# InSilicoModellingGroup/rdcFEs

Measured on AMD Instinct MI355X. Metric: elements_assembled_per_sec, higher is better.
Workload: dtype f64; 1 GPU; PIHNA TET4 K(119): 10110954 tets, 1728000 nodes, 5 unknowns, params run/PIHNA/input.dat (shipped), order=lex, state of SURVEY App. C (background (0,0,0,7170,0) of the shipped field file, tumour values inside a sphere r = 0.25; see state_sensitivity); scatter=rowgather, kernel_variant=auto, parallelism=single GPU, rank0_local_elements=10110954, rank0_nnz=639395950

## Files before the change

rdcfes_amd/csrc/rdc_capi.hip:

```cpp
#include <algorithm>
#include <cmath>
#include <cstdarg>
#include <cstdio>
#include <cstring>
#include <new>
#include <type_traits>

#include "rdc_internal.h"
#include "rdc_tet4_pihna_moments.h"
#include "rdc_tet4_ev.h"
#include "rdc_solid.h"

using namespace rdc;

namespace {

struct DevBuf {
  void* p = nullptr;
  size_t bytes = 0;
  bool owned = true;
};

thread_local char g_create_error[512] = "";

// ... 386 lines not shown
    a.rg2.sdesc = (const HostPrep::StoreDesc*)c->rg2_sdesc.p;
    a.rg2.contrib = (const uint16_t*)c->rg2_contrib.p;
    a.rg2.pair_aux = (const uint16_t*)c->rg2_aux.p;
    a.rg2.node_tab = (const uint16_t*)c->rg2_ntab.p;
    if (c->prep.rg4_nl_stride > 0) {
      a.rg2.nlist = (const uint32_t*)c->rg4_nlist.p;
      a.rg2.pair_loc = (const uint32_t*)c->rg4_ploc.p;
      a.rg2.nl_stride = c->prep.rg4_nl_stride;
      if ((M::NELEM > 0 || M::AUX_LOCAL_NODE >= 0) && !c->prep.pair_eid.empty()) {
        if (!c->rg5_eid_ready) {
          if ((rc = dev_upload(c, c->rg5_eid, c->prep.pair_eid))) return rc;
          c->rg5_eid_ready = true;
        }
        a.rg2.pair_eid = (const uint32_t*)c->rg5_eid.p;
      }
    }
    a.rg2.lds_bytes = c->prep.rg2_lds_bytes;
    a.rg2.block = c->prep.rg2_block;
  }
  const bool evc_model = EvcEligible<M>::value && evc_wanted(p, c->opt_special != 0);
  if (evc_model && a.nen == 4 && !c->ev_tried && c->prep.rg2_ok && c->opt_kernel == 0 && a.strategy == RDC_SCATTER_ROWGATHER && a.variant != RDC_VARIANT_GENERIC) {
    std::vector<uint32_t> conn_h((size_t)c->prep.n_elem * 4);
    RDC_HIP(c, hipMemcpyAsync(conn_h.data(), c->conn.p, conn_h.size() * sizeof(uint32_t), hipMemcpyDeviceToHost, c->stream));
    RDC_HIP(c, hipStreamSynchronize(c->stream));
    if ((rc = build_ev_lists(c, conn_h.data()))) return rc;
  }
  a.use_ev = c->prep_ev.ok && (c->opt_kernel == 0 || c->opt_kernel == 7) && c->opt_moments && (!c->opt_ablate || c->opt_kernel == 7) &&
             (!c->stamps.p || (c->opt_kernel == 7 && c->opt_ablate == 4)) && c->opt_occ != 1 && c->opt_ldspad == 0;
  a.opt_ev_occ = c->opt_ev_occ;
  a.opt_evc_occ = c->opt_evc_occ;
  a.opt_ev_resident = c->opt_ev_resident;
  a.opt_ev_bg = c->opt_ev_bg;
  if (c->opt_ev_resident) {
    if ((rc = dev_alloc(c, c->ev_ticket, 256))) return rc;
    a.ev_ticket = (int*)c->ev_ticket.p;
  }
  a.ev_grid = c->opt_grid > 0 ? c->opt_grid : 2 * c->n_cu;
  if (c->opt_kernel == 5 || c->opt_kernel == 7) a.opt_kernel = 0;
  if (a.use_ev) {
    a.ev.n_wg = (int)c->prep_ev.desc.size();
    a.ev.desc = (const HostPrepEv::Desc*)c->ev_desc.p;
    a.ev.nlist = (const uint32_t*)c->ev_nlist.p;
    a.ev.vloc = (const uint32_t*)c->ev_vloc.p;
    a.ev.vslot = (const uint32_t*)c->ev_vslot.p;
    a.ev.ntab = (const HostPrepEv::Node*)c->ev_ntab.p;
    a.ev.bpart = (const uint8_t*)c->ev_bpart.p;
    a.ev.nls = c->prep_ev.nls;
    a.ev.max_out_doubles = c->prep_ev.max_out_doubles;
  }
  bool hex_cl = false;
  if (a.nen == 8 && (M::NV == 3 || M::NV == 5) && c->opt_hex_kernel != 1 && (c->opt_part == 0 || c->opt_hex_kernel == 0) &&
      a.strategy == RDC_SCATTER_ROWGATHER && c->opt_solid_cl_waves == 31) {
    if ((rc = ensure_cluster_lists(c, 0))) return rc;
    hex_cl = c->solid_cl_state == 1;
  }
  bool pattern_ok = evc_model;
  if constexpr (std::is_same<M, Pihna>::value) pattern_ok = pihna_pattern_applies(p) || c->opt_ev_general;
  const bool ev_path = a.use_ev && (std::is_same<M, Pihna>::value || evc_model) && a.nen == 4 && a.variant != RDC_VARIANT_GENERIC &&
                       (c->opt_special || c->opt_ev_general || !std::is_same<M, Pihna>::value) && a.strategy == RDC_SCATTER_ROWGATHER && pattern_ok;
  if constexpr (std::is_same<M, Pihna>::value) a.ev_general = ev_path && c->opt_ev_general && !(c->opt_special && pihna_pattern_applies(p));
  if (!std::is_same<M, Pihna>::value) a.use_ev = ev_path && c->opt_kernel == 0;
  if (c->opt_part != 0 && ev_path) {
    if (c->opt_interior < 0) return fail(c, RDC_ERR_STATE, "\"part\" needs \"interior_nodes\"");
    if ((rc = ev_order_for_interior(c))) return rc;
    a.ev.wg_perm = (const uint32_t*)c->ev_perm.p;
    if (c->opt_part == 1) {
      c->part1_packed = false;
      c->part1_nodes = 0;
      if (c->ev_part1_wg == 0) return RDC_OK;
      c->part1_nodes = ev_part1_node_bound(c);
      a.ev.wg_begin = 0; a.ev.wg_count = c->ev_part1_wg;
      if (!c->pack_event) RDC_HIP(c, hipEventCreateWithFlags(&c->pack_event, hipEventDisableTiming));
      a.pack_part = 1; a.pack_event = c->pack_event;
      c->part1_packed = true;
    } else {
      a.ev.wg_begin = c->ev_part1_wg; a.ev.wg_count = -1;
      if (c->part1_packed) { a.pack_part = 2; a.pack_event = c->pack_event; }
      c->part1_packed = false;
    }
  } else
  if (c->opt_part != 0 && hex_cl) {
    c->part1_packed = false;
    if (c->opt_part == 1) {
      c->part1_nodes = c->scl_interior >= 0 ? c->scl_part1_nodes : 0;
      if (c->scl_interior < 0 || c->scl_n_wg_interior == 0) { c->part1_nodes = 0; return RDC_OK; }
    }
    a.cl = cluster_view(c, c->scl_interior >= 0 ? c->opt_part : (c->opt_part == 2 ? 0 : 1));
    if (a.cl.n_wg == 0) return RDC_OK;
  } else
  if (c->opt_part != 0) {
    const bool sub = a.nen == 4 && a.strategy == RDC_SCATTER_ROWGATHER && a.variant != RDC_VARIANT_GENERIC && a.rg2.n_wg > 0 &&
                     a.rg2.pair_aux && a.rg2.nlist && a.rg2.block == 256 && a.opt_kernel == 0 && c->opt_interior >= 0 &&
                     ((M::NELEM == 0 && M::AUX_LOCAL_NODE < 0) || a.rg2.pair_eid);
    const int split = sub ? part1_workgroups(c) : 0;
    if (c->opt_part == 1) {
      c->part1_packed = false;
      c->part1_nodes = 0;
      if (!sub || split == 0) return RDC_OK;
      c->part1_nodes = (int64_t)c->prep.wg2[(size_t)split - 1].n0 + c->prep.wg2[(size_t)split - 1].nnodes;
      a.rg2.wg_begin = 0; a.rg2.wg_count = split;
      if (!c->pack_event) RDC_HIP(c, hipEventCreateWithFlags(&c->pack_event, hipEventDisableTiming));
      a.pack_part = 1; a.pack_event = c->pack_event;
      c->part1_packed = true;
    } else {
      a.rg2.wg_begin = split; a.rg2.wg_count = -1;
      if (sub && c->part1_packed) { a.pack_part = 2; a.pack_event = c->pack_event; }
      c->part1_packed = false;
    }
  } else {
    c->part1_packed = false;
  }
  if (hex_cl && c->opt_part == 0) {
    a.cl = cluster_view(c);
    a.cl.grid = c->opt_hex_kernel == 2 ? 2 * c->n_cu : 0;
  }
  a.val = (double*)c->val.p;
  a.rhs = (double*)c->rhs.p;
  a.stream = c->stream;
  a.colour_ptr = c->prep.colour_ptr.data();
  a.n_colours = c->prep.n_colours;
  a.n_wg = c->prep.rowgather_ok ? (int)c->prep.wg_node_ptr.size() - 1 : 0;
  a.lds_bytes = c->prep.rg_lds_bytes;
  a.ev_start = nullptr;
  hipEvent_t ev_stop = nullptr;
  if (c->timing) {
    if ((rc = next_event_pair(c, &a.ev_start, &ev_stop))) return rc;
  }
  hipError_t e = launch_specialised<M>(a, k, *p);
  if (e != hipSuccess) return fail(c, RDC_ERR_HIP, "kernel launch failed: %s", hipGetErrorString(e));
  if (c->timing) RDC_HIP(c, hipEventRecord(ev_stop, c->stream));
  return RDC_OK;
}

template <class F>
int with_part(rdc_ctx* c, int part, void* stream, F&& call) {
  if (!c) return RDC_ERR_INVALID;
  if (part < 0 || part > 2) return fail(c, RDC_ERR_INVALID, "part must be 0, 1 or 2");
  const int part0 = c->opt_part;
  const hipStream_t s0 = c->stream;
  c->opt_part = part;
  c->stream = (hipStream_t)stream;
  const int rc = call();
  c->opt_part = part0;
  c->stream = s0;
  return rc;
}
}

extern "C" {

int rdc_abi_version(void) { return RDC_ABI_VERSION; }

const char* rdc_last_error(const rdc_ctx* ctx) { return ctx ? ctx->err : g_create_error; }

int rdc_device_count(int* n) {
  if (!n) return RDC_ERR_INVALID;
  int ndev = 0;
  const hipError_t e = hipGetDeviceCount(&ndev);
  *n = e == hipSuccess ? ndev : 0;
  return e == hipSuccess ? RDC_OK : fail(nullptr, RDC_ERR_HIP, "hipGetDeviceCount failed: %s", hipGetErrorString(e));
}

// ... 867 lines not shown
```

rdcfes_amd/csrc/rdc_internal.h:

```cpp
#ifndef RDC_INTERNAL_H
#define RDC_INTERNAL_H

#include <hip/hip_runtime.h>
#include <stdint.h>
#include <atomic>
#include <string>
#include <type_traits>
#include <vector>

#include "rdc_kernels.h"
#include "rdc_prep.h"

namespace rdc {

inline void dyn_lds_once(std::atomic<uint64_t>& done, const void* fn, int bytes) {
  int dev = 0;
  (void)hipGetDevice(&dev);
  const uint64_t bit = dev >= 0 && dev < 64 ? (1ull << dev) : 0;
  if (bit && (done.load(std::memory_order_relaxed) & bit)) return;
  (void)hipFuncSetAttribute(fn, hipFuncAttributeMaxDynamicSharedMemorySize, bytes);
  if (bit) done.fetch_or(bit, std::memory_order_relaxed);
}

struct Rg2Dev {
// ... 34 lines not shown
  const HostPrepCl::Node* ntab = nullptr;
  const uint32_t* eid = nullptr;
  const uint32_t* pair = nullptr;
  const uint32_t* pslot = nullptr;
  size_t max_row_doubles = 0;
  int grid = 0;
};

struct LaunchArgs {
  MeshDev m;
  int nen, exp_mode, strategy;
  const double* u;
  const double* aux;
  const int64_t* hx_nl_ptr = nullptr;
  const uint32_t* hx_nlist = nullptr;
  const uint16_t* hx_ploc = nullptr;
  int hx_max_nodes = 0;
  int opt_staged = 1;
  const double* elem = nullptr;
  double* packed;
  int pack_part = 0;
  hipEvent_t pack_event = nullptr;
  int variant;
  int opt_occ, opt_ablate, opt_kernel, opt_special, opt_xcd, opt_grid, opt_pf, opt_moments = 1, opt_stagger = 0, opt_ldspad = 0;
  Rg2Dev rg2;
  EvDev ev;
  ClDev cl;
  bool use_ev = false;
  int opt_ev_occ = 3;
  int opt_evc_occ = 2;
  int ev_grid = 0;
  int opt_ev_bg = 1;
  int* ev_ticket = nullptr;
  bool ev_general = false;
  int opt_ev_resident = 1;
  long long* stamps = nullptr;
  double* val;
  double* rhs;
  hipStream_t stream;
  hipEvent_t ev_start;
  const int64_t* colour_ptr;
  int n_colours;
  int n_wg;
  size_t lds_bytes;
};

template <class M>
hipError_t launch_rd(const LaunchArgs& a, const typename M::K& k);
template <class M>
hipError_t launch_tet4_fast(const LaunchArgs& a, const typename M::K& k);
hipError_t pack_nodes_pihna(const LaunchArgs& a);
hipError_t launch_tet4_ev(const LaunchArgs& a, const PihnaK& k);
template <class M>
hipError_t launch_tet4_evc(const LaunchArgs& a, const typename M::K& k);
template <class M> struct EvcEligible { static constexpr bool value = std::is_same<M, Ripf>::value; };

}
#endif
```

rdcfes_amd/csrc/rdc_tet4_ev.hip:

```cpp
#include "rdc_internal.h"
#include <type_traits>
#include "rdc_tet4_ev.h"

namespace rdc {

template <class M> struct RecEv {
  static constexpr int RAW = 3 + M::NV + M::NAUX;
  static constexpr int N = (RAW + 1) & ~1;
};

template <int ABL_>
struct EvSink {
  static constexpr int ABL = ABL_ == 4 ? 0 : ABL_;
  double* p[4][4];
  double* pr[4];
  double sum = 0.0;
  __device__ __forceinline__ void mom(int m, int i, int j, double v) {
    if (ABL == 0) __hip_atomic_fetch_add(p[i][j] + m * ev::NBP, v, __ATOMIC_RELAXED, __HIP_MEMORY_SCOPE_WORKGROUP);
    else if (ABL == 1) p[i][j][m * ev::NBP] = v;
    else sum += v;
  }
  __device__ __forceinline__ void rhs(int a, int i, double v) {
    if (ABL == 0) __hip_atomic_fetch_add(pr[i] + a * ev::MAXN, v, __ATOMIC_RELAXED, __HIP_MEMORY_SCOPE_WORKGROUP);
    else if (ABL == 1) pr[i][a * ev::MAXN] = v;
    else sum += v;
  }
};


template <int EXP_MODE, int MINW, int ABL = 0, bool GEN = false>
__global__ void __launch_bounds__(256, MINW)
k_tet4_ev(const HostPrepEv::Desc* __restrict__ desc, const uint32_t* __restrict__ nlist, const uint32_t* __restrict__ vloc,
          const uint32_t* __restrict__ vslot, const HostPrepEv::Node* __restrict__ ntab, const uint8_t* __restrict__ bpart,
          const uint32_t* __restrict__ wg_perm, const PihnaK k, const double* __restrict__ rec, double* __restrict__ val,
          double* __restrict__ rhs, const int nls, const int wg_begin, const int xcd_n, const int stagger,
          long long* __restrict__ stamps, const int bg_skip) {
  constexpr int BLOCK = 256, NP = 4;
  constexpr bool TL = ABL == 4;
  long long ts[11];
#define RDC_TS(x) if (TL) ts[x] = __builtin_amdgcn_s_memtime()
  RDC_TS(0);
  constexpr int NM = GEN ? ev::NMG : ev::NM, NBP = ev::NBP, MAXN = ev::MAXN;
  extern __shared__ __attribute__((aligned(16))) double lds[];
  __shared__ HostPrepEv::Node snode[MAXN];
  typedef __attribute__((address_space(3))) void* lds_ptr;
  typedef const __attribute__((address_space(1))) void* glb_ptr;
  if (stagger > 0 && blockIdx.x < 1024u) {
    const unsigned lds_base = __builtin_amdgcn_s_getreg((7 << 11) | 6);
    const uint32_t slot = lds_base == 0 ? 0u : (lds_base < 144u ? 1u : 2u);
    for (uint32_t i = 0; i < slot * (uint32_t)stagger; i++) __builtin_amdgcn_s_sleep(16);
  }
  int wl = (int)blockIdx.x;
  if (xcd_n > 0) {
    const int q = xcd_n >> 3, rem = xcd_n & 7, x = wl & 7;
    wl = x * q + (x < rem ? x : rem) + (wl >> 3);
  }
  int w = wl + wg_begin;
  if (wg_perm) w = (int)wg_perm[w];
  const int tid = threadIdx.x, lane = tid & 63, wv = tid >> 6;
  double* const R = lds + NM * NBP;
  double* const recs = R + 5 * MAXN;
  {
    static_assert((NM * NBP * 8) % (4 * 1024) == 0, "zeroing: 4 waves x (NM / 2) groups of four addtid stores of 256 bytes");
    constexpr int PER_WAVE = NM * NBP * 8 / 4;
    const uint32_t zbase = (uint32_t)(uintptr_t)lds + (uint32_t)__builtin_amdgcn_readfirstlane(wv) * (uint32_t)PER_WAVE;
    const uint32_t zero = 0u;
    uint32_t m0_saved;
    asm volatile("s_mov_b32 %0, m0\n\ts_mov_b32 m0, %1\n\ts_nop 0" : "=&s"(m0_saved) : "s"(zbase) : "memory");
#pragma unroll
    for (int o = 0; o < PER_WAVE; o += 1024)
      asm volatile("ds_write_addtid_b32 %0 offset:%1\n\tds_write_addtid_b32 %0 offset:%1+256\n\tds_write_addtid_b32 %0 offset:%1+512\n\tds_write_addtid_b32 %0 offset:%1+768"
                   :: "v"(zero), "n"(o) : "memory");
    asm volatile("s_mov_b32 m0, %0" :: "s"(m0_saved) : "memory");
    if (tid < 5 * MAXN) lds[NM * NBP + tid] = 0.0;
  }
  const int rounds = nls >> 6;
  uint32_t nid = 0;
  if (wv < rounds) nid = nlist[(size_t)w * nls + wv * 64 + lane];
  const uint32_t pl = vloc[(size_t)w * BLOCK + tid];
  const uint2 sl = reinterpret_cast<const uint2*>(vslot)[(size_t)w * BLOCK + tid];
  const HostPrepEv::Desc d = desc[w];
  const int mirror = (int)bpart[(size_t)w * NBP + tid];
  if (tid < MAXN) snode[tid] = ntab[(size_t)w * MAXN + tid];
  if (wv < rounds) {
    const char* src = reinterpret_cast<const char*>(rec) + (size_t)nid * (NP * 16);
#pragma unroll
    for (int p = 0; p < NP; p++)
      __builtin_amdgcn_global_load_lds((glb_ptr)(src + p * 16), (lds_ptr)(recs + (p * nls + wv * 64) * 2), 16, 0, 0);
  }
  RDC_TS(1);
  asm volatile("s_waitcnt vmcnt(0)" ::: "memory");
  RDC_TS(2);
  __syncthreads();
  RDC_TS(3);
  if (pl != 0xFFFFFFFFu) {
    double X[4][3], U[4][5];
    int li[4];
#pragma unroll
    for (int j = 0; j < 4; j++) {
      li[j] = (pl >> (8 * j)) & 0xFF;
      double rr[2 * NP];
#pragma unroll
      for (int p = 0; p < NP; p++) {
        const double2 v2 = reinterpret_cast<const double2*>(recs)[p * nls + li[j]];
        rr[2 * p] = v2.x; rr[2 * p + 1] = v2.y;
      }
      X[j][0] = rr[0]; X[j][1] = rr[1]; X[j][2] = rr[2];
#pragma unroll
      for (int v = 0; v < 5; v++) U[j][v] = rr[3 + v];
    }
    const int nown = (int)d.nown;
    const int r = (li[0] < nown) + (li[1] < nown) + (li[2] < nown) + (li[3] < nown);
    EvSink<ABL> sink;
    const uint32_t sw[4] = {sl.x & 0xFFFFu, sl.x >> 16, sl.y & 0xFFFFu, sl.y >> 16};
#pragma unroll
    for (int i = 0; i < 4; i++) {
      const int a = (i < r) ? li[i] : 0;
      sink.pr[i] = R + a;
#pragma unroll
      for (int j = 0; j < 4; j++) sink.p[i][j] = lds + a + MAXN * (int)((sw[i] >> (4 * j)) & 0xF);
    }
// ... 37 lines not shown
  RDC_TS(7);
  __syncthreads();
  RDC_TS(8);
  for (int n = wv; n < (int)d.nown; n += 4) {
    const HostPrepEv::Node nd = snode[n];
    const int cnt = 25 * (int)nd.len;
    double* out = val + (size_t)25 * nd.bptr;
    const double* img = lds + nd.obase;
    const int sh = (int)(nd.obase & 1);
    typedef double v2d_t __attribute__((ext_vector_type(2)));
    const int npair = (cnt - sh) >> 1;
    const v2d_t* src = reinterpret_cast<const v2d_t*>(img + sh);
    v2d_t* dstg = reinterpret_cast<v2d_t*>(out + sh);
    for (int x = lane; x < npair; x += 64) __builtin_nontemporal_store(src[x], dstg + x);
    if (sh && lane == 0) __builtin_nontemporal_store(img[0], out);
    if (((cnt - sh) & 1) && lane == 1) __builtin_nontemporal_store(img[cnt - 1], out + cnt - 1);
  }
  if (TL) {
    RDC_TS(9);
    if (stagger == 0) asm volatile("s_waitcnt vmcnt(0)" ::: "memory");
    RDC_TS(10);
    if (lane == 0 && stamps) {
      long long* o = stamps + ((int64_t)blockIdx.x * 4 + wv) * 12;
#pragma unroll
      for (int x = 0; x < 11; x++) o[x] = ts[x];
      o[11] = (long long)__builtin_amdgcn_s_getreg((31 << 11) | 4) | ((long long)__builtin_amdgcn_s_getreg((31 << 11) | 20) << 32);
    }
  }
#undef RDC_TS
}


namespace {
__device__ __forceinline__ void evl_dma16(const void* g, const void* lds_base) {
  const uint32_t b = __builtin_amdgcn_readfirstlane((uint32_t)(uintptr_t)lds_base);
  asm volatile("s_mov_b32 m0, %1\n\ts_nop 0\n\tglobal_load_lds_dwordx4 %0, off" ::"v"(g), "s"(b) : "memory", "m0");
}
}
namespace {
struct EvqLists {
  static constexpr int PL = 0, SL = 1024, MISC = SL + 2048, MIRROR = MISC, SNODE = MISC + 256, DESC = MISC + 512, NL = MISC + 544;
  static constexpr int bytes(int nls) { return NL + 2 * nls * 4; }
};
}
template <int EXP_MODE, bool TL, bool GEN = false>
__global__ void __launch_bounds__(256, GEN ? 2 : 3)
k_tet4_evq(const HostPrepEv::Desc* __restrict__ desc, const uint32_t* __restrict__ nlist, const uint32_t* __restrict__ vloc,
           const uint32_t* __restrict__ vslot, const HostPrepEv::Node* __restrict__ ntab, const uint8_t* __restrict__ bpart,
           const PihnaK k, const double* __restrict__ rec, double* __restrict__ val, double* __restrict__ rhs, const int nls,
           const int wg_begin, const int wg_count, long long* __restrict__ stamps, const int bg_skip, int* __restrict__ ticket,
           const uint32_t* __restrict__ wg_perm) {
  constexpr int BLOCK = 256, NP = 4;
  constexpr int NM = GEN ? ev::NMG : ev::NM, NBP = ev::NBP, MAXN = ev::MAXN;
  extern __shared__ __attribute__((aligned(16))) double lds[];
  __shared__ HostPrepEv::Node snode[MAXN];
  __shared__ uint8_t smirror[NBP];
  __shared__ int s_nown;
  __shared__ int s_tk[2];
  double* const R = lds + NM * NBP;
  double* const recs = R + 5 * MAXN;
  char* const lists = reinterpret_cast<char*>(recs + (size_t)NP * nls * 2);
  const int rounds = nls >> 6;
  auto lds_barrier = [&]() { asm volatile("s_waitcnt lgkmcnt(0)\n\ts_barrier" ::: "memory"); };
  const int wv = __builtin_amdgcn_readfirstlane((int)(threadIdx.x >> 6));
  constexpr int NONE = 0x7fffffff;
  int c0 = (int)blockIdx.x, c1 = c0 + (int)gridDim.x, c2 = c0 + 2 * (int)gridDim.x;
  auto cluster_of = [&](const int c) -> int { return c < wg_count ? (wg_perm ? (int)wg_perm[wg_begin + c] : wg_begin + c) : -1; };
  int w0c = cluster_of(c0), w1c = cluster_of(c1), w2c = cluster_of(c2);
  long long ts[8];
#define RDC_TS(x) if (TL) ts[x] = __builtin_amdgcn_s_memtime()
  auto fetch = [&](const int w, const uint32_t nid, const int w2, const int nb2, const int lane) {
    if (wv < rounds) {
      const char* src = reinterpret_cast<const char*>(rec) + (size_t)nid * (NP * 16);
#pragma unroll
      for (int p = 0; p < NP; p++) evl_dma16(src + p * 16, recs + (p * nls + wv * 64) * 2);
    }
    if (wv == 0) evl_dma16(reinterpret_cast<const char*>(vloc + (size_t)w * BLOCK) + lane * 16, lists + EvqLists::PL);
    else if (wv < 3) evl_dma16(reinterpret_cast<const char*>(vslot + (size_t)w * BLOCK * 2) + (wv - 1) * 1024 + lane * 16, lists + EvqLists::SL + (wv - 1) * 1024);
    else {
      if (lane < 34) {
        const char* src = lane < 16 ? reinterpret_cast<const char*>(bpart + (size_t)w * NBP) + lane * 16
                        : lane < 32 ? reinterpret_cast<const char*>(ntab + (size_t)w * MAXN) + (lane - 16) * 16
                                    : reinterpret_cast<const char*>(desc + w) + (lane - 32) * 16;
        evl_dma16(src, lists + EvqLists::MISC);
      }
      if (w2 >= 0 && lane < (nls >> 2)) evl_dma16(reinterpret_cast<const char*>(nlist + (size_t)w2 * nls) + lane * 16, lists + EvqLists::NL + nb2 * nls * 4);
    }
  };
  {
    uint32_t nid0 = 0;
    if (wv < rounds) nid0 = nlist[(size_t)w0c * nls + threadIdx.x];
    asm volatile("s_waitcnt vmcnt(0)" : "+v"(nid0)::"memory");
    fetch(w0c, nid0, w1c, 1, (int)(threadIdx.x & 63));
  }
  int tk = NONE;
  bool pending = false;
#pragma unroll 1
  for (int it = 0;; it++) {
    int lane;
    asm volatile("v_mbcnt_lo_u32_b32 %0, -1, 0\n\tv_mbcnt_hi_u32_b32 %0, -1, %0" : "=v"(lane));
    const int w = w0c;
    RDC_TS(0);
    {
      constexpr int PER_WAVE = NM * NBP * 8 / 4;
      const uint32_t zbase = (uint32_t)(uintptr_t)lds + (uint32_t)wv * (uint32_t)PER_WAVE;
      const uint32_t zero = 0u;
      uint32_t m0_saved;
      asm volatile("s_mov_b32 %0, m0\n\ts_mov_b32 m0, %1\n\ts_nop 0" : "=&s"(m0_saved) : "s"(zbase) : "memory");
#pragma unroll
      for (int o = 0; o < PER_WAVE; o += 1024)
        asm volatile("ds_write_addtid_b32 %0 offset:%1\n\tds_write_addtid_b32 %0 offset:%1+256\n\tds_write_addtid_b32 %0 offset:%1+512\n\tds_write_addtid_b32 %0 offset:%1+768"
                     :: "v"(zero), "n"(o) : "memory");
      asm volatile("s_mov_b32 m0, %0" :: "s"(m0_saved) : "memory");
      if (wv * 64 + lane < 5 * MAXN) lds[NM * NBP + wv * 64 + lane] = 0.0;
    }
    asm volatile("s_waitcnt vmcnt(0)" : "+v"(tk)::"memory");
    if (pending && wv == 0 && lane == 0) s_tk[0] = tk == NONE ? NONE : 3 * (int)gridDim.x + tk;
    RDC_TS(1);
    lds_barrier();
    RDC_TS(2);
    if (pending) { c2 = __builtin_amdgcn_readfirstlane(s_tk[0]); w2c = cluster_of(c2); }
    if (c0 >= wg_count) break;
    {
      const int tid = wv * 64 + lane;
      const uint32_t pl = *reinterpret_cast<const uint32_t*>(lists + EvqLists::PL + tid * 4);
      const uint2 sl = *reinterpret_cast<const uint2*>(lists + EvqLists::SL + tid * 8);
      const int nown = (int)reinterpret_cast<const HostPrepEv::Desc*>(lists + EvqLists::DESC)->nown;
      {
        const int blk = (((wv & 1) << 3) | (lane >> 3)) * MAXN + (((wv >> 1) << 3) | (lane & 7));
        smirror[blk] = *reinterpret_cast<const uint8_t*>(lists + EvqLists::MIRROR + blk);
        if (tid < MAXN) snode[tid] = *reinterpret_cast<const HostPrepEv::Node*>(lists + EvqLists::SNODE + tid * 16);
        if (tid == 0) s_nown = nown;
      }
      if (pl != 0xFFFFFFFFu) {
        double X[4][3], U[4][5];
        int li[4];
#pragma unroll
        for (int j = 0; j < 4; j++) {
          li[j] = (pl >> (8 * j)) & 0xFF;
          double rr[2 * NP];
#pragma unroll
          for (int p = 0; p < NP; p++) {
            const double2 v2 = reinterpret_cast<const double2*>(recs)[p * nls + li[j]];
            rr[2 * p] = v2.x; rr[2 * p + 1] = v2.y;
          }
          X[j][0] = rr[0]; X[j][1] = rr[1]; X[j][2] = rr[2];
#pragma unroll
          for (int v = 0; v < 5; v++) U[j][v] = rr[3 + v];
        }
        const int r = (li[0] < nown) + (li[1] < nown) + (li[2] < nown) + (li[3] < nown);
        EvSink<0> sink;
        const uint32_t sw[4] = {sl.x & 0xFFFFu, sl.x >> 16, sl.y & 0xFFFFu, sl.y >> 16};
#pragma unroll
        for (int i = 0; i < 4; i++) {
          const int a = (i < r) ? li[i] : 0;
          sink.pr[i] = R + a;
#pragma unroll
          for (int j = 0; j < 4; j++) sink.p[i][j] = lds + a + MAXN * (int)((sw[i] >> (4 * j)) & 0xF);
        }
        const bool bg = bg_skip && __builtin_amdgcn_ballot_w64(!ev::pihna_background(U)) == 0;
        ev::pihna_visit<EXP_MODE, EvSink<0>, true, GEN>(k, X, U, r, sink, bg);
      }
    }
    RDC_TS(3);
    lds_barrier();
    RDC_TS(4);
    asm volatile("v_mbcnt_lo_u32_b32 %0, -1, 0\n\tv_mbcnt_hi_u32_b32 %0, -1, %0" : "=v"(lane));
    if (c1 < wg_count) {
      uint32_t nid = 0;
      if (wv < rounds) nid = *reinterpret_cast<const uint32_t*>(lists + EvqLists::NL + (((it + 1) & 1) * nls + wv * 64 + lane) * 4);
      fetch(w1c, nid, w2c, it & 1, lane);
    }
    tk = NONE;
    if (c2 < wg_count && wv == 0 && lane == 0) {
      const int one = 1;
      asm volatile("global_atomic_add %0, %1, %2, off sc0" : "=v"(tk) : "v"(ticket), "v"(one) : "memory");
    }
    pending = true;
    const int nown = s_nown;
    const int bn = ((wv >> 1) << 3) | (lane & 7), bs = ((wv & 1) << 3) | (lane >> 3), blk = bs * MAXN + bn;
    double e[NM];
    const bool has = bn < nown && bs < (int)snode[bn < nown ? bn : 0].len;
#pragma unroll
    for (int m = 0; m < NM; m++) e[m] = 0.0;
    if (has) {
      const int mirror = (int)smirror[blk];
#pragma unroll
      for (int m = 0; m < NM; m++) e[m] = lds[m * NBP + blk];
      if (mirror != blk) {
#pragma unroll
        for (int m = 0; m < NM; m++)
          if (GEN ? ev::symmetric_moment_gen(m) : ev::symmetric_moment(m)) e[m] += lds[m * NBP + mirror];
      }
    }
    {
      const int tid = wv * 64 + lane;
      if (tid < nown * 5) {
        const int n = tid / 5, a = tid - n * 5;
        rhs[(size_t)snode[n].node * 5 + a] = R[a * MAXN + n];
      }
    }
    double o[25];
    ev::pihna_expand(k, e, o);
    lds_barrier();
// ... 8 lines not shown
#pragma unroll
        for (int a = 0; a < 5; a++)
#pragma unroll
          for (int b = 0; b < 5; b++) dst[a * len5 + b] = o[a * 5 + b];
      }
      lds_barrier();
      const int n1 = nown < n0 + 8 ? nown : n0 + 8;
      for (int n = n0 + wv; n < n1; n += 4) {
        const HostPrepEv::Node nd = snode[n];
        const int cnt = 25 * (int)nd.len;
        double* out = val + (size_t)25 * nd.bptr;
        const double* img = lds + (nd.obase - base);
        const int sh = (int)(nd.obase & 1);
        typedef double v2d_t __attribute__((ext_vector_type(2)));
        const int npair = (cnt - sh) >> 1;
        const v2d_t* src = reinterpret_cast<const v2d_t*>(img + sh);
        v2d_t* dstg = reinterpret_cast<v2d_t*>(out + sh);
        for (int x = lane; x < npair; x += 64) __builtin_nontemporal_store(src[x], dstg + x);
        if (sh && lane == 0) __builtin_nontemporal_store(img[0], out);
        if (((cnt - sh) & 1) && lane == 1) __builtin_nontemporal_store(img[cnt - 1], out + cnt - 1);
      }
      lds_barrier();
    }
    RDC_TS(5);
    if (TL && lane == 0 && stamps) {
      long long* op = stamps + ((int64_t)c0 * 4 + wv) * 12;
#pragma unroll
      for (int x = 0; x < 6; x++) op[x] = ts[x];
      op[11] = (long long)__builtin_amdgcn_s_getreg((31 << 11) | 4) | ((long long)__builtin_amdgcn_s_getreg((31 << 11) | 20) << 32);
    }
    c0 = c1; c1 = c2; w0c = w1c; w1c = w2c;
  }
#undef RDC_TS
}


hipError_t launch_tet4_ev(const LaunchArgs& a, const PihnaK& k) {
  const EvDev& E = a.ev;
  hipError_t e = pack_nodes_pihna(a);
  if (e != hipSuccess) return e;
  if (a.ev_start) (void)hipEventRecord(a.ev_start, a.stream);
  const int wg_count = E.wg_count < 0 ? E.n_wg - E.wg_begin : E.wg_count;
  if (wg_count <= 0) return hipSuccess;
  const size_t acc = (size_t)(a.ev_general ? ev::NMG : ev::NM) * ev::NBP + 5 * ev::MAXN + (size_t)4 * E.nls * 2;
  const size_t lds_doubles = acc > E.max_out_doubles ? acc : E.max_out_doubles;
  const size_t lds_bytes = lds_doubles * sizeof(double);
  const int evq_grid = a.opt_grid > 0 ? a.opt_grid : (a.ev_grid > 0 ? (a.ev_general ? a.ev_grid : a.ev_grid / 2 * 3) : 768);
  if (a.opt_ev_resident && (!a.opt_ablate || (a.opt_ablate == 4 && !a.ev_general)) && a.opt_ev_occ == 3 && !a.opt_xcd && a.opt_stagger == 0 &&
      (a.opt_grid > 0 || a.opt_ev_resident == 2 || (int64_t)wg_count >= 56 * (int64_t)evq_grid)) {
    int grid = evq_grid;
    if (grid > wg_count) grid = wg_count;
    const size_t bytes = ((size_t)(a.ev_general ? ev::NMG : ev::NM) * ev::NBP + 5 * ev::MAXN + (size_t)4 * E.nls * 2) * sizeof(double) + EvqLists::bytes(E.nls);
    if (!a.ev_ticket) return hipErrorInvalidValue;
#define RDC_EVQ(MODE, TLV, GENV)                                                                                                              \
  hipLaunchKernelGGL((k_tet4_evq<MODE, TLV, GENV>), dim3(grid), dim3(256), bytes, a.stream, E.desc, E.nlist, E.vloc, E.vslot, E.ntab, E.bpart, k, \
                     a.packed, a.val, a.rhs, E.nls, E.wg_begin, wg_count, a.stamps, a.opt_ev_bg, a.ev_ticket + (a.pack_part == 2 ? 16 : 0), E.wg_perm)
    if (a.ev_general) { if (a.exp_mode == 3) RDC_EVQ(3, false, true); else RDC_EVQ(0, false, true); }
    else if (a.opt_ablate == 4) { if (a.exp_mode == 3) RDC_EVQ(3, true, false); else RDC_EVQ(0, true, false); }
    else { if (a.exp_mode == 3) RDC_EVQ(3, false, false); else RDC_EVQ(0, false, false); }
#undef RDC_EVQ
    return hipGetLastError();
  }
#define RDC_EV(MODE, MINW)                                                                                          \
  hipLaunchKernelGGL((k_tet4_ev<MODE, MINW>), dim3(wg_count), dim3(256), lds_bytes, a.stream, E.desc, E.nlist, E.vloc, \
                     E.vslot, E.ntab, E.bpart, E.wg_perm, k, a.packed, a.val, a.rhs, E.nls, E.wg_begin, a.opt_xcd ? wg_count : 0, a.opt_stagger, a.stamps, a.opt_ev_bg)
  if (a.exp_mode == 3 && a.opt_ablate >= 1 && a.opt_ablate <= 4 && !a.ev_general) {
#define RDC_EVA(X)                                                                                                    \
  hipLaunchKernelGGL((k_tet4_ev<3, 3, X>), dim3(wg_count), dim3(256), lds_bytes, a.stream, E.desc, E.nlist, E.vloc, \
                     E.vslot, E.ntab, E.bpart, E.wg_perm, k, a.packed, a.val, a.rhs, E.nls, E.wg_begin, a.opt_xcd ? wg_count : 0, a.opt_stagger, a.stamps, a.opt_ev_bg)
    if (a.opt_ablate == 1) RDC_EVA(1); else if (a.opt_ablate == 2) RDC_EVA(2); else if (a.opt_ablate == 3) RDC_EVA(3); else RDC_EVA(4);
#undef RDC_EVA
    return hipGetLastError();
  }
  if (a.ev_general) {
#define RDC_EVG(MODE)                                                                                                       \
  hipLaunchKernelGGL((k_tet4_ev<MODE, 2, 0, true>), dim3(wg_count), dim3(256), lds_bytes, a.stream, E.desc, E.nlist, E.vloc, \
                     E.vslot, E.ntab, E.bpart, E.wg_perm, k, a.packed, a.val, a.rhs, E.nls, E.wg_begin, a.opt_xcd ? wg_count : 0, a.opt_stagger, a.stamps, a.opt_ev_bg)
    if (a.exp_mode == 3) RDC_EVG(3); else RDC_EVG(0);
#undef RDC_EVG
    return hipGetLastError();
  }
  if (a.exp_mode == 3) { if (a.opt_ev_occ == 2) RDC_EV(3, 2); else RDC_EV(3, 3); }
  else { if (a.opt_ev_occ == 2) RDC_EV(0, 2); else RDC_EV(0, 3); }
#undef RDC_EV
  return hipGetLastError();
}

}
```

rdcfes_amd/csrc/rdc_tet4_fast.hip:

```cpp
#include "rdc_internal.h"
#include "rdc_tet4_fast.h"
#include "rdc_tet4_pihna_moments.h"

#include <type_traits>

namespace rdc {

template <class M> struct Rec {
  static constexpr int NA = M::NAUX;
  static constexpr int RAW = 3 + M::NV + NA;
  static constexpr int N = (RAW + 1) & ~1;
};

template <class M>
__global__ void k_pack_nodes(int64_t node_begin, int64_t node_end, const double* __restrict__ xyz, const double* __restrict__ u,
                             const double* __restrict__ aux, double* __restrict__ rec, int* __restrict__ ticket) {
  constexpr int N = Rec<M>::N, NV = M::NV, NA = M::NAUX;
  if (ticket && blockIdx.x == 0 && threadIdx.x == 0) *ticket = 0;
  const int64_t stride = (int64_t)gridDim.x * blockDim.x;
  for (int64_t t = node_begin * N + (int64_t)blockIdx.x * blockDim.x + threadIdx.x; t < node_end * N; t += stride) {
    const int64_t n = t / N;
    const int c = (int)(t - n * N);
    double v = 0.0;
    if (c < 3) v = xyz[3 * n + c];
    else if (c < 3 + NV) v = u[n * NV + (c - 3)];
    else if (c < 3 + NV + NA) v = aux[n * (NA > 0 ? NA : 1) + (c - 3 - NV)];
    rec[t] = v;
  }
}

template <class M>
__device__ __forceinline__ void load_rec(const double* __restrict__ rec, int64_t n, double (&X)[3], double (&U)[M::NV],
                                         double (&A)[M::NAUX > 0 ? M::NAUX : 1]) {
  constexpr int N = Rec<M>::N, NV = M::NV, NA = M::NAUX;
  const double2* p = reinterpret_cast<const double2*>(rec + n * N);
  double r[N];
#pragma unroll
  for (int x = 0; x < N / 2; x++) { const double2 v = p[x]; r[2 * x] = v.x; r[2 * x + 1] = v.y; }
  X[0] = r[0]; X[1] = r[1]; X[2] = r[2];
#pragma unroll
  for (int v = 0; v < NV; v++) U[v] = r[3 + v];
  if (NA > 0) {
#pragma unroll
    for (int v = 0; v < NA; v++) A[v] = r[3 + NV + v];
  } else {
    A[0] = 0.0;
  }
}

template <class M> RDC_HD constexpr bool block_nonzero(int a, int b) {
  bool any = M::hasA(a, b) || M::hasD(a, b);
// ... 437 lines not shown
    if (I >= m.n_owned) continue;
    double X[4][3], U[4][NV], AX[4][M::NAUX > 0 ? M::NAUX : 1];
    RmwSink<M> sink;
#pragma unroll
    for (int j = 0; j < 4; j++) {
      const int jo = j ^ i;
      const int64_t n = m.conn[e * 4 + jo];
      load_rec<M>(rec, n, X[j], U[j], AX[j]);
      if (M::AUX_LOCAL_NODE >= 0 && jo != M::AUX_LOCAL_NODE) {
#pragma unroll
        for (int v = 0; v < (M::NAUX > 0 ? M::NAUX : 1); v++) AX[j][v] = 0.0;
      }
      sink.off[j] = NV * (int64_t)m.eslot[e * 16 + i * 4 + jo];
      sink.first[j] = (fm >> (i * 4 + jo)) & 1ull;
    }
    const int64_t b0 = m.bptr[I];
    sink.stride = NV * (m.bptr[I + 1] - b0);
    sink.row = val + NV * NV * b0;
    sink.prhs = rhs + I * NV;
    sink.first_rhs = (fr >> i) & 1u;
    tet4_row0<M, EXP_MODE>(k, X, U, AX, sink, M::NELEM > 0 ? elem + e * M::NELEM : nullptr);
  }
}

template <class M>
static hipError_t pack_nodes(const LaunchArgs& a) {
  int64_t nb = 0, ne = a.m.n_node;
  if (a.pack_part == 1) ne = a.m.n_owned;
  else if (a.pack_part == 2) { nb = a.m.n_owned; if (a.pack_event) (void)hipStreamWaitEvent(a.stream, a.pack_event, 0); }
  const int64_t total = (ne - nb) * Rec<M>::N;
  if (total > 0) {
    int64_t grid = (total + 255) / 256;
    if (grid > 4096) grid = 4096;
    hipLaunchKernelGGL((k_pack_nodes<M>), dim3((unsigned)grid), dim3(256), 0, a.stream, nb, ne, a.m.xyz, a.u, a.aux, a.packed, a.ev_ticket ? a.ev_ticket + (a.pack_part == 2 ? 16 : 0) : nullptr);
  } else if (a.ev_ticket) {
    (void)hipMemsetAsync(a.ev_ticket + (a.pack_part == 2 ? 16 : 0), 0, sizeof(int), a.stream);
  }
  if (a.pack_part == 1 && a.pack_event) (void)hipEventRecord(a.pack_event, a.stream);
  return hipGetLastError();
}

hipError_t pack_nodes_pihna(const LaunchArgs& a) { return pack_nodes<Pihna>(a); }

template <class M, int EXP_MODE>
static hipError_t launch_fast_impl(const LaunchArgs& a, const typename M::K& k) {
  {
    const hipError_t pe = pack_nodes<M>(a);
    if (pe != hipSuccess) return pe;
  }
  if (a.ev_start) (void)hipEventRecord(a.ev_start, a.stream);
  if constexpr (EvcEligible<M>::value)
  if (a.use_ev && a.ev.n_wg > 0 && a.strategy == RDC_SCATTER_ROWGATHER) return launch_tet4_evc<M>(a, k);
  if (a.strategy == RDC_SCATTER_ROWGATHER && a.rg2.n_wg > 0 && a.rg2.pair_aux && a.rg2.nlist && a.rg2.block == 256 &&
      (a.opt_kernel == 0 || M::NELEM > 0 || M::AUX_LOCAL_NODE >= 0)) {
    constexpr int BLOCK = 256;
    const int nl = a.rg2.nl_stride;
    const int acc_doubles = (int)((a.rg2.lds_bytes / sizeof(double) + 3) & ~(size_t)1);
    const size_t lds_bytes = sizeof(double) * ((size_t)acc_doubles + (size_t)(Rec<M>::N / 2) * nl * 2) + (size_t)a.opt_ldspad * 1024;
    const int wg_begin = a.rg2.wg_begin, wg_count = a.rg2.wg_count < 0 ? a.rg2.n_wg - a.rg2.wg_begin : a.rg2.wg_count;
    if (wg_count <= 0) return hipSuccess;
#define RDC_RG5(MINW, ST)                                                                                          \
  hipLaunchKernelGGL((k_tet4_rg5<M, EXP_MODE, BLOCK, MINW, ST>), dim3(wg_count), dim3(BLOCK), lds_bytes, a.stream,     \
                     a.rg2.desc, a.rg2.pair_loc, a.rg2.pair_aux, a.rg2.nlist, a.rg2.node_tab, k, a.packed, a.val, a.rhs, \
                     nl, acc_doubles, a.stamps, a.opt_pf, a.opt_xcd, a.rg2.pair_eid, a.elem, wg_begin, a.opt_stagger)
    if constexpr ((std::is_same<M, PihnaNoCellTransport>::value || std::is_same<M, PihnaNoCellTransportMoments>::value) && EXP_MODE == 3) {
      if (a.opt_ablate >= 1 && a.opt_ablate <= 6) {
#define RDC_ABL(X)                                                                                                        \
  hipLaunchKernelGGL((k_tet4_rg5<M, EXP_MODE, BLOCK, 2, false, X>), dim3(wg_count), dim3(BLOCK), lds_bytes, a.stream,      \
                     a.rg2.desc, a.rg2.pair_loc, a.rg2.pair_aux, a.rg2.nlist, a.rg2.node_tab, k, a.packed, a.val, a.rhs, \
// ... 112 lines not shown
```

Baseline: 7.037 billion elements/s.

## Gather node data directly from xyz/u in EV kernels, dropping the pack pass

For the specialised PIHNA edge-vertex kernels, the per-call k_pack_nodes pass is skipped. Node coordinates and unknowns are instead gathered straight from the xyz and u arrays into LDS, using LDS-direct DMA loads plus a small register-staged piece. Resetting the work-stealing ticket moves from the pack kernel into the persistent kernel itself, which resets the counters when the last block finishes. This removes a full extra pass over the node data and a kernel launch each call. The cost is less regular, unaligned 16-byte gathers and more complex ticket-reset logic.

```diff
diff --git a/rdcfes_amd/csrc/rdc_capi.hip b/rdcfes_amd/csrc/rdc_capi.hip
--- a/rdcfes_amd/csrc/rdc_capi.hip
+++ b/rdcfes_amd/csrc/rdc_capi.hip
@@ -442,7 +442,11 @@
   a.opt_ev_resident = c->opt_ev_resident;
   a.opt_ev_bg = c->opt_ev_bg;
   if (c->opt_ev_resident) {
-    if ((rc = dev_alloc(c, c->ev_ticket, 256))) return rc;
+    if (!c->ev_ticket.p) {
+      if ((rc = dev_alloc(c, c->ev_ticket, 256))) return rc;
+      RDC_HIP(c, hipMemsetAsync(c->ev_ticket.p, 0, 256, c->stream));
+      RDC_HIP(c, hipStreamSynchronize(c->stream));
+    }
     a.ev_ticket = (int*)c->ev_ticket.p;
   }
   a.ev_grid = c->opt_grid > 0 ? c->opt_grid : 2 * c->n_cu;
@@ -480,11 +484,14 @@
       if (c->ev_part1_wg == 0) return RDC_OK;
       c->part1_nodes = ev_part1_node_bound(c);
       a.ev.wg_begin = 0; a.ev.wg_count = c->ev_part1_wg;
-      if (!c->pack_event) RDC_HIP(c, hipEventCreateWithFlags(&c->pack_event, hipEventDisableTiming));
-      a.pack_part = 1; a.pack_event = c->pack_event;
-      c->part1_packed = true;
+      if (!std::is_same<M, Pihna>::value || a.ev_general) {
+        if (!c->pack_event) RDC_HIP(c, hipEventCreateWithFlags(&c->pack_event, hipEventDisableTiming));
+        a.pack_part = 1; a.pack_event = c->pack_event;
+        c->part1_packed = true;
+      }
     } else {
       a.ev.wg_begin = c->ev_part1_wg; a.ev.wg_count = -1;
+      a.ev_part = 2;
       if (c->part1_packed) { a.pack_part = 2; a.pack_event = c->pack_event; }
       c->part1_packed = false;
     }
@@ -537,7 +544,10 @@
     if ((rc = next_event_pair(c, &a.ev_start, &ev_stop))) return rc;
   }
   hipError_t e = launch_specialised<M>(a, k, *p);
-  if (e != hipSuccess) return fail(c, RDC_ERR_HIP, "kernel launch failed: %s", hipGetErrorString(e));
+  if (e != hipSuccess) {
+    if (c->ev_ticket.p) (void)hipMemset(c->ev_ticket.p, 0, 256);
+    return fail(c, RDC_ERR_HIP, "kernel launch failed: %s", hipGetErrorString(e));
+  }
   if (c->timing) RDC_HIP(c, hipEventRecord(ev_stop, c->stream));
   return RDC_OK;
 }
diff --git a/rdcfes_amd/csrc/rdc_internal.h b/rdcfes_amd/csrc/rdc_internal.h
--- a/rdcfes_amd/csrc/rdc_internal.h
+++ b/rdcfes_amd/csrc/rdc_internal.h
@@ -90,6 +90,7 @@
   int ev_grid = 0;
   int opt_ev_bg = 1;
   int* ev_ticket = nullptr;
+  int ev_part = 0;
   bool ev_general = false;
   int opt_ev_resident = 1;
   long long* stamps = nullptr;
diff --git a/rdcfes_amd/csrc/rdc_tet4_ev.hip b/rdcfes_amd/csrc/rdc_tet4_ev.hip
--- a/rdcfes_amd/csrc/rdc_tet4_ev.hip
+++ b/rdcfes_amd/csrc/rdc_tet4_ev.hip
@@ -28,12 +28,52 @@
 };
 
 
+namespace {
+__device__ __forceinline__ void evl_dma16(const void* g, const void* lds_base) {
+  const uint32_t b = __builtin_amdgcn_readfirstlane((uint32_t)(uintptr_t)lds_base);
+  asm volatile("s_mov_b32 m0, %1\n\ts_nop 0\n\tglobal_load_lds_dwordx4 %0, off" ::"v"(g), "s"(b) : "memory", "m0");
+}
+__device__ __forceinline__ void evl_dma4(const void* g, const void* lds_base) {
+  const uint32_t b = __builtin_amdgcn_readfirstlane((uint32_t)(uintptr_t)lds_base);
+  asm volatile("s_mov_b32 m0, %1\n\ts_nop 0\n\tglobal_load_lds_dword %0, off" ::"v"(g), "s"(b) : "memory", "m0");
+}
+struct EvGather {
+  static constexpr int MAX64 = 3;
+  template <bool WAIT, class ID>
+  static __device__ __forceinline__ void run(ID id_at, const double* xyz, const double* u, double* recs, const int nls, const int w, const int lane) {
+    const int n64 = 3 * (nls >> 6);
+    uint32_t i64[MAX64];
+#pragma unroll
+    for (int x = 0; x < MAX64; x++) i64[x] = w + 4 * x < n64 ? id_at(64 * ((w + 4 * x) / 3) + lane) : 0u;
+    if (WAIT) asm volatile("s_waitcnt vmcnt(0)" : "+v"(i64[0]), "+v"(i64[1]), "+v"(i64[2])::"memory");
+#pragma unroll
+    for (int x = 0; x < MAX64; x++) {
+      const int t = w + 4 * x;
+      if (t < n64) {
+        const int gr = t / 3, pi = t - 3 * gr;
+        const char* src = pi == 0 ? reinterpret_cast<const char*>(xyz) + (size_t)i64[x] * 24
+                                  : reinterpret_cast<const char*>(u) + (size_t)i64[x] * 40 + (pi == 1 ? 8 : 24);
+        evl_dma16(src, recs + ((pi == 0 ? 0 : pi + 1) * nls + 64 * gr) * 2);
+      }
+    }
+  }
+  static __device__ __forceinline__ void piece1_load(const double* xyz, const double* u, const uint32_t nid, double& z, double& n) {
+    const char* az = reinterpret_cast<const char*>(xyz) + (size_t)nid * 24 + 16;
+    const char* an = reinterpret_cast<const char*>(u) + (size_t)nid * 40;
+    asm volatile("global_load_dwordx2 %0, %2, off\n\tglobal_load_dwordx2 %1, %3, off" : "=&v"(z), "=&v"(n) : "v"(az), "v"(an) : "memory");
+  }
+  static __device__ __forceinline__ void piece1_store(double* recs, const int nls, const int q, const double z, const double n) {
+    reinterpret_cast<double2*>(recs)[nls + q] = double2{z, n};
+  }
+};
+}
+
 template <int EXP_MODE, int MINW, int ABL = 0, bool GEN = false>
 __global__ void __launch_bounds__(256, MINW)
 k_tet4_ev(const HostPrepEv::Desc* __restrict__ desc, const uint32_t* __restrict__ nlist, const uint32_t* __restrict__ vloc,
           const uint32_t* __restrict__ vslot, const HostPrepEv::Node* __restrict__ ntab, const uint8_t* __restrict__ bpart,
-          const uint32_t* __restrict__ wg_perm, const PihnaK k, const double* __restrict__ rec, double* __restrict__ val,
-          double* __restrict__ rhs, const int nls, const int wg_begin, const int xcd_n, const int stagger,
+          const uint32_t* __restrict__ wg_perm, const PihnaK k, const double* __restrict__ xyz, const double* __restrict__ u,
+          const double* __restrict__ rec, double* __restrict__ val, double* __restrict__ rhs, const int nls, const int wg_begin, const int xcd_n, const int stagger,
           long long* __restrict__ stamps, const int bg_skip) {
   constexpr int BLOCK = 256, NP = 4;
   constexpr bool TL = ABL == 4;
@@ -43,8 +83,6 @@
   constexpr int NM = GEN ? ev::NMG : ev::NM, NBP = ev::NBP, MAXN = ev::MAXN;
   extern __shared__ __attribute__((aligned(16))) double lds[];
   __shared__ HostPrepEv::Node snode[MAXN];
-  typedef __attribute__((address_space(3))) void* lds_ptr;
-  typedef const __attribute__((address_space(1))) void* glb_ptr;
   if (stagger > 0 && blockIdx.x < 1024u) {
     const unsigned lds_base = __builtin_amdgcn_s_getreg((7 << 11) | 6);
     const uint32_t slot = lds_base == 0 ? 0u : (lds_base < 144u ? 1u : 2u);
@@ -74,19 +112,25 @@
     asm volatile("s_mov_b32 m0, %0" :: "s"(m0_saved) : "memory");
     if (tid < 5 * MAXN) lds[NM * NBP + tid] = 0.0;
   }
-  const int rounds = nls >> 6;
-  uint32_t nid = 0;
-  if (wv < rounds) nid = nlist[(size_t)w * nls + wv * 64 + lane];
   const uint32_t pl = vloc[(size_t)w * BLOCK + tid];
   const uint2 sl = reinterpret_cast<const uint2*>(vslot)[(size_t)w * BLOCK + tid];
   const HostPrepEv::Desc d = desc[w];
   const int mirror = (int)bpart[(size_t)w * NBP + tid];
   if (tid < MAXN) snode[tid] = ntab[(size_t)w * MAXN + tid];
-  if (wv < rounds) {
-    const char* src = reinterpret_cast<const char*>(rec) + (size_t)nid * (NP * 16);
-#pragma unroll
-    for (int p = 0; p < NP; p++)
-      __builtin_amdgcn_global_load_lds((glb_ptr)(src + p * 16), (lds_ptr)(recs + (p * nls + wv * 64) * 2), 16, 0, 0);
+  const uint32_t* nl0 = nlist + (size_t)w * nls;
+  if constexpr (GEN) {
+    uint32_t nid = 0;
+    if (tid < nls) nid = nl0[tid];
+    asm volatile("s_waitcnt vmcnt(0)" : "+v"(nid)::"memory");
+    if (tid < nls) {
+#pragma unroll
+      for (int p = 0; p < NP; p++) evl_dma16(reinterpret_cast<const char*>(rec) + (size_t)nid * (NP * 16) + p * 16, recs + (p * nls + (tid & ~63)) * 2);
+    }
+  } else {
+    uint32_t nid = 0;
+    if (tid < nls) nid = nl0[tid];
+    EvGather::run<true>([&](const int q) { return nl0[q]; }, xyz, u, recs, nls, __builtin_amdgcn_readfirstlane(wv), lane);
+    if (tid < nls) EvGather::piece1_store(recs, nls, tid, xyz[(size_t)nid * 3 + 2], u[(size_t)nid * 5]);
   }
   RDC_TS(1);
   asm volatile("s_waitcnt vmcnt(0)" ::: "memory");
@@ -190,12 +234,6 @@
 
 
 namespace {
-__device__ __forceinline__ void evl_dma16(const void* g, const void* lds_base) {
-  const uint32_t b = __builtin_amdgcn_readfirstlane((uint32_t)(uintptr_t)lds_base);
-  asm volatile("s_mov_b32 m0, %1\n\ts_nop 0\n\tglobal_load_lds_dwordx4 %0, off" ::"v"(g), "s"(b) : "memory", "m0");
-}
-}
-namespace {
 struct EvqLists {
   static constexpr int PL = 0, SL = 1024, MISC = SL + 2048, MIRROR = MISC, SNODE = MISC + 256, DESC = MISC + 512, NL = MISC + 544;
   static constexpr int bytes(int nls) { return NL + 2 * nls * 4; }
@@ -205,7 +243,8 @@
 __global__ void __launch_bounds__(256, GEN ? 2 : 3)
 k_tet4_evq(const HostPrepEv::Desc* __restrict__ desc, const uint32_t* __restrict__ nlist, const uint32_t* __restrict__ vloc,
            const uint32_t* __restrict__ vslot, const HostPrepEv::Node* __restrict__ ntab, const uint8_t* __restrict__ bpart,
-           const PihnaK k, const double* __restrict__ rec, double* __restrict__ val, double* __restrict__ rhs, const int nls,
+           const PihnaK k, const double* __restrict__ xyz, const double* __restrict__ u, const double* __restrict__ rec, double* __restrict__ val,
+           double* __restrict__ rhs, const int nls,
            const int wg_begin, const int wg_count, long long* __restrict__ stamps, const int bg_skip, int* __restrict__ ticket,
            const uint32_t* __restrict__ wg_perm) {
   constexpr int BLOCK = 256, NP = 4;
@@ -218,7 +257,6 @@
   double* const R = lds + NM * NBP;
   double* const recs = R + 5 * MAXN;
   char* const lists = reinterpret_cast<char*>(recs + (size_t)NP * nls * 2);
-  const int rounds = nls >> 6;
   auto lds_barrier = [&]() { asm volatile("s_waitcnt lgkmcnt(0)\n\ts_barrier" ::: "memory"); };
   const int wv = __builtin_amdgcn_readfirstlane((int)(threadIdx.x >> 6));
   constexpr int NONE = 0x7fffffff;
@@ -227,12 +265,8 @@
   int w0c = cluster_of(c0), w1c = cluster_of(c1), w2c = cluster_of(c2);
   long long ts[8];
 #define RDC_TS(x) if (TL) ts[x] = __builtin_amdgcn_s_memtime()
-  auto fetch = [&](const int w, const uint32_t nid, const int w2, const int nb2, const int lane) {
-    if (wv < rounds) {
-      const char* src = reinterpret_cast<const char*>(rec) + (size_t)nid * (NP * 16);
-#pragma unroll
-      for (int p = 0; p < NP; p++) evl_dma16(src + p * 16, recs + (p * nls + wv * 64) * 2);
-    }
+  double p1z = 0.0, p1n = 0.0;
+  auto fetch = [&](const int w, const int w2, const int nb2, const int lane) {
     if (wv == 0) evl_dma16(reinterpret_cast<const char*>(vloc + (size_t)w * BLOCK) + lane * 16, lists + EvqLists::PL);
     else if (wv < 3) evl_dma16(reinterpret_cast<const char*>(vslot + (size_t)w * BLOCK * 2) + (wv - 1) * 1024 + lane * 16, lists + EvqLists::SL + (wv - 1) * 1024);
     else {
@@ -245,12 +279,20 @@
       if (w2 >= 0 && lane < (nls >> 2)) evl_dma16(reinterpret_cast<const char*>(nlist + (size_t)w2 * nls) + lane * 16, lists + EvqLists::NL + nb2 * nls * 4);
     }
   };
+  auto fetch_packed = [&](const uint32_t nid, const int lane) {
+#pragma unroll
+    for (int p = 0; p < NP; p++) evl_dma16(reinterpret_cast<const char*>(rec) + (size_t)nid * (NP * 16) + p * 16, recs + (p * nls + wv * 64) * 2);
+  };
   {
-    uint32_t nid0 = 0;
-    if (wv < rounds) nid0 = nlist[(size_t)w0c * nls + threadIdx.x];
-    asm volatile("s_waitcnt vmcnt(0)" : "+v"(nid0)::"memory");
-    fetch(w0c, nid0, w1c, 1, (int)(threadIdx.x & 63));
-  }
+    const uint32_t* nl0 = nlist + (size_t)w0c * nls;
+    if constexpr (!GEN) EvGather::run<true>([&](const int q) { return nl0[q]; }, xyz, u, recs, nls, wv, (int)(threadIdx.x & 63));
+    if ((int)threadIdx.x < nls) {
+      uint32_t nid = nl0[threadIdx.x];
+      asm volatile("s_waitcnt vmcnt(0)" : "+v"(nid)::"memory");
+      if constexpr (GEN) fetch_packed(nid, (int)(threadIdx.x & 63)); else EvGather::piece1_load(xyz, u, nid, p1z, p1n);
+    }
+  }
+  fetch(w0c, w1c, 1, (int)(threadIdx.x & 63));
   int tk = NONE;
   bool pending = false;
 #pragma unroll 1
@@ -272,7 +314,9 @@
       asm volatile("s_mov_b32 m0, %0" :: "s"(m0_saved) : "memory");
       if (wv * 64 + lane < 5 * MAXN) lds[NM * NBP + wv * 64 + lane] = 0.0;
     }
-    asm volatile("s_waitcnt vmcnt(0)" : "+v"(tk)::"memory");
+    asm volatile("s_waitcnt vmcnt(0)" : "+v"(tk), "+v"(p1z), "+v"(p1n)::"memory");
+    if (!GEN && c0 < wg_count && wv * 64 + lane < nls) EvGather::piece1_store(recs, nls, wv * 64 + lane, p1z, p1n);
+    p1z = p1n = 0.0;
     if (pending && wv == 0 && lane == 0) s_tk[0] = tk == NONE ? NONE : 3 * (int)gridDim.x + tk;
     RDC_TS(1);
     lds_barrier();
@@ -325,9 +369,16 @@
     RDC_TS(4);
     asm volatile("v_mbcnt_lo_u32_b32 %0, -1, 0\n\tv_mbcnt_hi_u32_b32 %0, -1, %0" : "=v"(lane));
     if (c1 < wg_count) {
-      uint32_t nid = 0;
-      if (wv < rounds) nid = *reinterpret_cast<const uint32_t*>(lists + EvqLists::NL + (((it + 1) & 1) * nls + wv * 64 + lane) * 4);
-      fetch(w1c, nid, w2c, it & 1, lane);
+      const uint32_t* idb = reinterpret_cast<const uint32_t*>(lists + EvqLists::NL) + ((it + 1) & 1) * nls;
+      int nls_g, wv_g;
+      asm volatile("s_mov_b32 %0, %2\n\ts_mov_b32 %1, %3" : "=s"(nls_g), "=s"(wv_g) : "s"(nls), "s"(wv));
+      if constexpr (GEN) {
+        if (wv_g * 64 + lane < nls_g) fetch_packed(idb[wv_g * 64 + lane], lane);
+      } else {
+        EvGather::run<false>([&](const int q) { return idb[q]; }, xyz, u, recs, nls_g, wv_g, lane);
+        if (wv_g * 64 + lane < nls_g) EvGather::piece1_load(xyz, u, idb[wv_g * 64 + lane], p1z, p1n);
+      }
+      fetch(w1c, w2c, it & 1, lane);
     }
     tk = NONE;
     if (c2 < wg_count && wv == 0 && lane == 0) {
@@ -402,13 +453,24 @@
     c0 = c1; c1 = c2; w0c = w1c; w1c = w2c;
   }
 #undef RDC_TS
+  int lane_end;
+  asm volatile("v_mbcnt_lo_u32_b32 %0, -1, 0\n\tv_mbcnt_hi_u32_b32 %0, -1, %0" : "=v"(lane_end));
+  if (wv == 0 && lane_end == 0) {
+    const int left = __hip_atomic_fetch_add(ticket + 1, 1, __ATOMIC_RELAXED, __HIP_MEMORY_SCOPE_AGENT);
+    if (left == (int)gridDim.x - 1) {
+      (void)__hip_atomic_exchange(ticket, 0, __ATOMIC_RELAXED, __HIP_MEMORY_SCOPE_AGENT);
+      (void)__hip_atomic_exchange(ticket + 1, 0, __ATOMIC_RELAXED, __HIP_MEMORY_SCOPE_AGENT);
+    }
+  }
 }
 
 
 hipError_t launch_tet4_ev(const LaunchArgs& a, const PihnaK& k) {
   const EvDev& E = a.ev;
-  hipError_t e = pack_nodes_pihna(a);
-  if (e != hipSuccess) return e;
+  if (a.ev_general) {
+    const hipError_t e = pack_nodes_pihna(a);
+    if (e != hipSuccess) return e;
+  }
   if (a.ev_start) (void)hipEventRecord(a.ev_start, a.stream);
   const int wg_count = E.wg_count < 0 ? E.n_wg - E.wg_begin : E.wg_count;
   if (wg_count <= 0) return hipSuccess;
@@ -424,7 +486,7 @@
     if (!a.ev_ticket) return hipErrorInvalidValue;
 #define RDC_EVQ(MODE, TLV, GENV)                                                                                                              \
   hipLaunchKernelGGL((k_tet4_evq<MODE, TLV, GENV>), dim3(grid), dim3(256), bytes, a.stream, E.desc, E.nlist, E.vloc, E.vslot, E.ntab, E.bpart, k, \
-                     a.packed, a.val, a.rhs, E.nls, E.wg_begin, wg_count, a.stamps, a.opt_ev_bg, a.ev_ticket + (a.pack_part == 2 ? 16 : 0), E.wg_perm)
+                     a.m.xyz, a.u, a.packed, a.val, a.rhs, E.nls, E.wg_begin, wg_count, a.stamps, a.opt_ev_bg, a.ev_ticket + (a.ev_part == 2 ? 16 : 0), E.wg_perm)
     if (a.ev_general) { if (a.exp_mode == 3) RDC_EVQ(3, false, true); else RDC_EVQ(0, false, true); }
     else if (a.opt_ablate == 4) { if (a.exp_mode == 3) RDC_EVQ(3, true, false); else RDC_EVQ(0, true, false); }
     else { if (a.exp_mode == 3) RDC_EVQ(3, false, false); else RDC_EVQ(0, false, false); }
@@ -433,11 +495,11 @@
   }
 #define RDC_EV(MODE, MINW)                                                                                          \
   hipLaunchKernelGGL((k_tet4_ev<MODE, MINW>), dim3(wg_count), dim3(256), lds_bytes, a.stream, E.desc, E.nlist, E.vloc, \
-                     E.vslot, E.ntab, E.bpart, E.wg_perm, k, a.packed, a.val, a.rhs, E.nls, E.wg_begin, a.opt_xcd ? wg_count : 0, a.opt_stagger, a.stamps, a.opt_ev_bg)
+                     E.vslot, E.ntab, E.bpart, E.wg_perm, k, a.m.xyz, a.u, a.packed, a.val, a.rhs, E.nls, E.wg_begin, a.opt_xcd ? wg_count : 0, a.opt_stagger, a.stamps, a.opt_ev_bg)
   if (a.exp_mode == 3 && a.opt_ablate >= 1 && a.opt_ablate <= 4 && !a.ev_general) {
 #define RDC_EVA(X)                                                                                                    \
   hipLaunchKernelGGL((k_tet4_ev<3, 3, X>), dim3(wg_count), dim3(256), lds_bytes, a.stream, E.desc, E.nlist, E.vloc, \
-                     E.vslot, E.ntab, E.bpart, E.wg_perm, k, a.packed, a.val, a.rhs, E.nls, E.wg_begin, a.opt_xcd ? wg_count : 0, a.opt_stagger, a.stamps, a.opt_ev_bg)
+                     E.vslot, E.ntab, E.bpart, E.wg_perm, k, a.m.xyz, a.u, a.packed, a.val, a.rhs, E.nls, E.wg_begin, a.opt_xcd ? wg_count : 0, a.opt_stagger, a.stamps, a.opt_ev_bg)
     if (a.opt_ablate == 1) RDC_EVA(1); else if (a.opt_ablate == 2) RDC_EVA(2); else if (a.opt_ablate == 3) RDC_EVA(3); else RDC_EVA(4);
 #undef RDC_EVA
     return hipGetLastError();
@@ -445,7 +507,7 @@
   if (a.ev_general) {
 #define RDC_EVG(MODE)                                                                                                       \
   hipLaunchKernelGGL((k_tet4_ev<MODE, 2, 0, true>), dim3(wg_count), dim3(256), lds_bytes, a.stream, E.desc, E.nlist, E.vloc, \
-                     E.vslot, E.ntab, E.bpart, E.wg_perm, k, a.packed, a.val, a.rhs, E.nls, E.wg_begin, a.opt_xcd ? wg_count : 0, a.opt_stagger, a.stamps, a.opt_ev_bg)
+                     E.vslot, E.ntab, E.bpart, E.wg_perm, k, a.m.xyz, a.u, a.packed, a.val, a.rhs, E.nls, E.wg_begin, a.opt_xcd ? wg_count : 0, a.opt_stagger, a.stamps, a.opt_ev_bg)
     if (a.exp_mode == 3) RDC_EVG(3); else RDC_EVG(0);
 #undef RDC_EVG
     return hipGetLastError();
diff --git a/rdcfes_amd/csrc/rdc_tet4_fast.hip b/rdcfes_amd/csrc/rdc_tet4_fast.hip
--- a/rdcfes_amd/csrc/rdc_tet4_fast.hip
+++ b/rdcfes_amd/csrc/rdc_tet4_fast.hip
@@ -14,9 +14,8 @@
 
 template <class M>
 __global__ void k_pack_nodes(int64_t node_begin, int64_t node_end, const double* __restrict__ xyz, const double* __restrict__ u,
-                             const double* __restrict__ aux, double* __restrict__ rec, int* __restrict__ ticket) {
+                             const double* __restrict__ aux, double* __restrict__ rec) {
   constexpr int N = Rec<M>::N, NV = M::NV, NA = M::NAUX;
-  if (ticket && blockIdx.x == 0 && threadIdx.x == 0) *ticket = 0;
   const int64_t stride = (int64_t)gridDim.x * blockDim.x;
   for (int64_t t = node_begin * N + (int64_t)blockIdx.x * blockDim.x + threadIdx.x; t < node_end * N; t += stride) {
     const int64_t n = t / N;
@@ -520,9 +519,7 @@
   if (total > 0) {
     int64_t grid = (total + 255) / 256;
     if (grid > 4096) grid = 4096;
-    hipLaunchKernelGGL((k_pack_nodes<M>), dim3((unsigned)grid), dim3(256), 0, a.stream, nb, ne, a.m.xyz, a.u, a.aux, a.packed, a.ev_ticket ? a.ev_ticket + (a.pack_part == 2 ? 16 : 0) : nullptr);
-  } else if (a.ev_ticket) {
-    (void)hipMemsetAsync(a.ev_ticket + (a.pack_part == 2 ? 16 : 0), 0, sizeof(int), a.stream);
+    hipLaunchKernelGGL((k_pack_nodes<M>), dim3((unsigned)grid), dim3(256), 0, a.stream, nb, ne, a.m.xyz, a.u, a.aux, a.packed);
   }
   if (a.pack_part == 1 && a.pack_event) (void)hipEventRecord(a.pack_event, a.stream);
   return hipGetLastError();
```

Measured after the change: 7.150 billion elements/s (median of 6 runs). +1.6%, better.
